# JINXER000/GIE-mapping

Measured on AMD Instinct MI355X. Metric: edt_map_update_throughput, higher is better.
Workload: dtype int32; 1 GPU; 512x512x512 @ 0.05 m, sensor-less hash world (BASELINE config 5): occupied iff hash(x,y,z) < 1 %, full observation, 25 ~; preset=c5, fast_mode=False, tiles=single volume, blocks=360448

## Files before the change

gie-mapping_amd/csrc/gie_hip.hip:

```cpp
#include <cstdio>
#include <unistd.h>
#include <cstring>
#include <cstdlib>
#include <string>
#include <algorithm>
#include <vector>
#include <hip/hip_runtime.h>
#include <hip/hip_ext.h>
#include <rocprim/rocprim.hpp>
#include "gie_kernels.hip.h"

#define GIE_NEV 8

struct be_state {
    int device;
    int num_cu;
    int cu_total;
    hipStream_t stream;
    hipEvent_t ev[GIE_NEV];
    int ev_set[GIE_NEV];
    void *scan_tmp; size_t scan_bytes;
    void *arena;
    hipEvent_t copy_ev[2];
    hipStream_t side;
// ... 267 lines not shown
}
static void be_exclusive_scan(be_state *b, const int32_t *flag, int32_t *rank, int n)
{
    size_t bytes = 0;
    (void)hipSetDevice(b->device);
    GIE_HIP_OK(rocprim::exclusive_scan(nullptr, bytes, flag, rank, 0, (size_t)n, rocprim::plus<int32_t>(), b->stream));
    if (bytes > b->scan_bytes) {
        if (b->scan_tmp) { (void)hipStreamSynchronize(b->stream); (void)hipFree(b->scan_tmp); }
        GIE_HIP_OK(hipMalloc(&b->scan_tmp, bytes)); b->scan_bytes = bytes;
    }
    GIE_HIP_OK(rocprim::exclusive_scan(b->scan_tmp, bytes, flag, rank, 0, (size_t)n, rocprim::plus<int32_t>(), b->stream));
}

template <int CP, int TX, int WAVES> static void gie_launch_edt_z(be_state *b, const gie_ctx &c, int full)
{
    constexpr int LP = 64 * CP;
    const size_t tile = ((size_t)c.Z * (TX + 1) + 3) & ~(size_t)3;
    const size_t lds = tile * 4 + (size_t)WAVES * LP * 8 + (size_t)LP * 2 + 16;
    static bool attr_done = false;
    if (!attr_done) {
        GIE_HIP_OK(hipFuncSetAttribute(reinterpret_cast<const void *>(&k_edt_z<CP, TX, WAVES>), hipFuncAttributeMaxDynamicSharedMemorySize, 160 * 1024));
        attr_done = true;
    }
    const int ntx = (c.X + TX - 1) / TX, ntiles = ntx * c.Y;
    int wgs = (int)((160 * 1024) / (lds + 256));
    if (wgs < 1) wgs = 1; if (wgs > 4) wgs = 4;
    int grid = wgs * b->cu_total; if (grid > (ntiles + 1) / 2) grid = (ntiles + 1) / 2;
    GIE_LAUNCH(b, (k_edt_z<CP, TX, WAVES>), dim3(grid), dim3(64 * WAVES), lds, c, ntx, ntiles, full);
}
template <int CP> static void gie_launch_edt_xz(be_state *b, const gie_ctx &c, bool zpass, int full, int zs_fused = 0, bool redo = false)
{
    if (redo) {
        GIE_LAUNCH(b, k_edt_x_redo<CP>, dim3(b->cu_total * 8), dim3(64 * GIE_EDTX_WAVES), 0, c);
    } else if (!zpass) {
        GIE_LAUNCH(b, k_edt_x<CP>, dim3((c.Y + GIE_EDTX_WAVES - 1) / GIE_EDTX_WAVES, c.Z), dim3(64 * GIE_EDTX_WAVES), 0, c, zs_fused, full);
    } else {
        gie_launch_edt_z<CP, 16, 8>(b, c, full);
    }
}
static void gie_launch_edt_dim(be_state *b, const gie_ctx &c, int L, bool zpass, int full, int zs_fused = 0, bool redo = false)
{
    if (L <= 64) gie_launch_edt_xz<1>(b, c, zpass, full, zs_fused, redo);
    else if (L <= 128) gie_launch_edt_xz<2>(b, c, zpass, full, zs_fused, redo);
    else if (L <= 256) gie_launch_edt_xz<4>(b, c, zpass, full, zs_fused, redo);
    else if (L <= 512) gie_launch_edt_xz<8>(b, c, zpass, full, zs_fused, redo);
    else gie_launch_edt_xz<16>(b, c, zpass, full, zs_fused, redo);
}
static int be_zs_mode(const gie_ctx &c)
{
    if (c.Z < 64 || c.Z > 1024) return 0;
    static const int on = GIE_SWITCH("GIE_ZSTREAM", 1);
    static const int fused = GIE_SWITCH("GIE_ZS_FUSED", 1);
    return on ? ((fused && (c.X & 1) == 0) ? 2 : 1) : 0;
}
static int be_edt_z_stream(be_state *b, const gie_ctx &c, int full);
static void be_edt_z_rest(be_state *b, const gie_ctx &c, int full, int zs)
{
    if (zs == 2) gie_launch_edt_dim(b, c, c.X, false, full, 0, true);
    gie_launch_edt_dim(b, c, c.Z, true, full);
}
static void be_edt_z(be_state *b, const gie_ctx &c, int full) { be_edt_z_rest(b, c, full, be_edt_z_stream(b, c, full) ? be_zs_mode(c) : 0); }
template <bool STAGED, class F> static void be_vox_list(be_state *b, const gie_ctx &c, const F &f, const int32_t *list, int count_idx, int always_list, int lx = 64)
{
    static const int mult = GIE_SWITCH("GIE_VOXA_MULT", 32);
    const dim3 g(b->cu_total * mult), t(256);
    if (lx == 32) GIE_LAUNCH(b, (k_voxa<F, STAGED, 32>), g, t, 0, c, f, list, count_idx, always_list);
    else if (lx == 16) GIE_LAUNCH(b, (k_voxa<F, STAGED, 16>), g, t, 0, c, f, list, count_idx, always_list);
    else if (lx == 8) GIE_LAUNCH(b, (k_voxa<F, STAGED, 8>), g, t, 0, c, f, list, count_idx, always_list);
    else GIE_LAUNCH(b, (k_voxa<F, STAGED, 64>), g, t, 0, c, f, list, count_idx, always_list);
}
static void be_markc(be_state *b, const gie_ctx &c, const int32_t *list)
{
    static const int generic = GIE_SWITCH("GIE_MARKC_GENERIC", 0);
    static const int lx = GIE_SWITCH("GIE_MARKC_LX", 32);
    static const int mult = GIE_SWITCH("GIE_VOXA_MULT", 64);
    if (generic) { be_vox_list<true>(b, c, op_markc(), list, GIE_CNT_TL_KNOWN, 0, lx == 16 || lx == 8 || lx == 32 ? lx : 64); return; }
    static const int lmult = GIE_SWITCH("GIE_MARKC_LGRID", 40);
    const dim3 g(b->cu_total * ((c.coc_defer && c.lazy_ok) ? lmult : mult)), t(256);
    if (lx == 16) GIE_LAUNCH(b, k_markc<16>, g, t, 0, c, list);
    else if (lx == 64) GIE_LAUNCH(b, k_markc<64>, g, t, 0, c, list);
    else GIE_LAUNCH(b, k_markc<32>, g, t, 0, c, list);
}
static float be_place_probe(be_state *b, const gie_ctx &c, int reps, int streams = 15)
{
    static const int mult = GIE_SWITCH("GIE_VOXA_MULT", 64);
    const long long ntile = (long long)c.tfd[0] * c.tfd[1] * c.tfd[2];
    const int nslot = (int)(ntile < c.max_blocks ? ntile : c.max_blocks);
    hipEvent_t e0, e1;
    if (hipEventCreate(&e0) != hipSuccess || hipEventCreate(&e1) != hipSuccess) return -1.f;
    std::vector<float> ms;
    hipLaunchKernelGGL(k_place_probe, dim3(b->cu_total * mult), dim3(256), 0, b->stream, c, nslot, streams);
    for (int r = 0; r < reps; r++) {
        (void)hipEventRecord(e0, b->stream);
        hipLaunchKernelGGL(k_place_probe, dim3(b->cu_total * mult), dim3(256), 0, b->stream, c, nslot, streams);
        (void)hipEventRecord(e1, b->stream);
        (void)hipEventSynchronize(e1);
        float t = 0.f; (void)hipEventElapsedTime(&t, e0, e1); ms.push_back(t);
    }
    (void)hipEventDestroy(e0); (void)hipEventDestroy(e1);
    std::sort(ms.begin(), ms.end());
    GIE_HIP_OK(hipMemsetAsync(c.pair, 0, (size_t)c.N * sizeof(uint64_t), b->stream));
    return ms.empty() ? -1.f : ms[ms.size() / 2];
}
static int be_rows_mode() { static const int v = GIE_SWITCH("GIE_ROWS", 1); return v ? 2 : 0; }
static void be_fuse(be_state *b, const gie_ctx &c, const int32_t *list)
{
    static const int mult = GIE_SWITCH("GIE_ROWS_MULT", 32);
    if (be_rows_mode()) {
        if (c.pntcld_mode) GIE_LAUNCH(b, k_fuse_rows<true>, dim3(b->cu_total * mult), dim3(256), 0, c, op_fuse(), list);
        else GIE_LAUNCH(b, k_fuse_rows<false>, dim3(b->cu_total * mult), dim3(256), 0, c, op_fuse(), list);
    }
    else be_vox_list<true>(b, c, op_fuse(), list, GIE_CNT_TL_FUSE, 0);
}
static void be_frontier_tiles(be_state *b, const gie_ctx &c, const int32_t *known, int known_idx, const int32_t *list, int count_idx)
{
    gie_face_patches fp;
    const int da[6] = { c.Y, c.Y, c.X, c.X, c.X, c.X }, db[6] = { c.Z, c.Z, c.Z, c.Z, c.Y, c.Y };
    fp.off[0] = 0;
    for (int f = 0; f < 6; f++) { fp.na[f] = (da[f] + 7) / 8; fp.off[f + 1] = fp.off[f] + fp.na[f] * ((db[f] + 7) / 8); }
    const long long ntile = (long long)c.tfd[0] * c.tfd[1] * c.tfd[2];
    int nsum = (int)((ntile + 64 * GIE_FF_WAVES - 1) / (64 * GIE_FF_WAVES));
    if (nsum > 2 * b->cu_total) nsum = 2 * b->cu_total;
    const int nface = (fp.off[6] + GIE_FF_WAVES - 1) / GIE_FF_WAVES;
    GIE_LAUNCH(b, k_frontier_faces, dim3(nsum + nface), dim3(64 * GIE_FF_WAVES), 0, c, fp, known, known_idx, nsum);
    static int mult = GIE_SWITCH("GIE_FRONT_MULT", 0);
    if (mult <= 0) {
        int per_cu = 0;
        if (hipOccupancyMaxActiveBlocksPerMultiprocessor(&per_cu, reinterpret_cast<const void *>(&k_frontier_tiles), 64 * GIE_FR_WAVES, 0) != hipSuccess || per_cu < 1) per_cu = 2;
        mult = per_cu;
    }
    GIE_LAUNCH(b, k_frontier_tiles, dim3(b->cu_total * mult), dim3(64 * GIE_FR_WAVES), 0, c, list, count_idx);
}
static void be_edt_z_direct(be_state *b, const gie_ctx &c)
{
    GIE_LAUNCH(b, k_edt_z_direct, dim3(b->cu_total * 16), dim3(256), 0, c);
}
static int be_edt_z_stream(be_state *b, const gie_ctx &c, int full)
{
    const int zs = be_zs_mode(c);
    if (!zs) return 0;
    const int nxr = (c.X + 63) / 64;
    static const int target = GIE_SWITCH("GIE_ZSTREAM_WAVES", 8);
    const long long want = (long long)b->cu_total * 4 * target;
    int nseg = (int)((want + (long long)nxr * c.Y - 1) / ((long long)nxr * c.Y));
    const int maxseg = c.Z / 64 > 0 ? c.Z / 64 : 1;
    if (nseg > maxseg) nseg = maxseg; if (nseg < 1) nseg = 1;
    int seg_len = ((c.Z + nseg - 1) / nseg + 31) & ~31;
    nseg = (c.Z + seg_len - 1) / seg_len;
    const long long waves = (long long)nxr * nseg * c.Y;
    long long grid = (waves + 3) / 4;
    const long long cap = (long long)b->cu_total * 8 * 4;
    if (grid > cap) grid = cap;
    if (!full && grid < (long long)b->cu_total * 16) grid = (long long)b->cu_total * 16;
    if (zs == 2) GIE_LAUNCH(b, k_edt_z_stream<true>, dim3((unsigned)grid), dim3(256), 0, c, full, nseg, seg_len, zs);
    else GIE_LAUNCH(b, k_edt_z_stream<false>, dim3((unsigned)grid), dim3(256), 0, c, full, nseg, seg_len, zs);
    return 1;
}
static void be_tile_oldskip(be_state *b, const gie_ctx &c, const int pupvt[3])
{
    const int ntile = c.tfd[0] * c.tfd[1] * c.tfd[2];
    int32_t *const count = &c.cnt[GIE_CNT_STATE1];
    GIE_LAUNCH(b, k_tile_oldskip, dim3((ntile + 255) / 256), dim3(256), 0, c, ntile, c.wc_list[0], count);
    if (c.catchup_fast) GIE_LAUNCH(b, k_coc_catchup_new, dim3(b->cu_total * 8), dim3(256), 0, c, pupvt[0], pupvt[1], pupvt[2], c.wc_list[0], count);
}
static void be_pair_materialise(be_state *b, const gie_ctx &c, int stay)
{
    const int ntile = c.tfd[0] * c.tfd[1] * c.tfd[2];
    int32_t *const count = &c.cnt[GIE_CNT_STATE2];
    GIE_LAUNCH(b, k_pair_lazy_list, dim3((ntile + 255) / 256), dim3(256), 0, c, ntile, stay, c.wc_list[1], count);
    GIE_LAUNCH(b, k_pair_lazy_run, dim3(b->cu_total * 8), dim3(256), 0, c, c.wc_list[1], count);
}
static void be_coc_catchup(be_state *b, const gie_ctx &c, const gie_catchup &p)
{
    const int ntile = c.tfd[0] * c.tfd[1] * c.tfd[2];
    int32_t *const count = &c.cnt[GIE_CNT_STATE1];
    GIE_HIP_OK(hipMemsetAsync(count, 0, sizeof(int32_t), b->stream));
    GIE_LAUNCH(b, k_coc_catchup_list, dim3((ntile + 255) / 256), dim3(256), 0, c, p, ntile, c.wc_list[0], count);
    GIE_LAUNCH(b, k_coc_catchup_run, dim3(b->cu_total * 4), dim3(256), 0, c, p, c.wc_list[0], count);
}
static void be_edt_prep(be_state *b, const gie_ctx &c)
{
    const int ncol = c.tfd[0] * c.tfd[1];
    GIE_LAUNCH(b, k_edt_prep, dim3((ncol + GIE_PREP_WAVES - 1) / GIE_PREP_WAVES), dim3(64 * GIE_PREP_WAVES), 0, c, ncol);
}
static void be_edt(be_state *b, const gie_ctx &c, int full)
{
    dim3 gy((c.X + GIE_EDTY_COLS - 1) / GIE_EDTY_COLS, c.Z);
    be_prof(b, 6, 0);
    static const int y4 = GIE_SWITCH("GIE_EDTY4", 1);
    if (y4 && (c.X & 3) == 0) {
        const int yb = c.Y > 512 ? 32 : 16, nq = (c.Y + yb - 1) / yb;
        const int lanes = (y4 == 3) ? 32 : 16;
        dim3 g4((c.X / 4 + lanes - 1) / lanes, c.Z), b4(lanes, nq);
        if (yb == 16 && lanes == 16) GIE_LAUNCH(b, (k_edt_y4<16, 16>), g4, b4, 0, c);
        else if (yb == 16) GIE_LAUNCH(b, (k_edt_y4<16, 32>), g4, b4, 0, c);
        else if (lanes == 16) GIE_LAUNCH(b, (k_edt_y4<32, 16>), g4, b4, 0, c);
        else GIE_LAUNCH(b, (k_edt_y4<32, 32>), g4, b4, 0, c);
    }
    else if (c.Y <= 256) GIE_LAUNCH(b, (k_edt_y<8, 8>), gy, dim3(GIE_EDTY_COLS, 8), 0, c);
    else if (c.Y <= 512) GIE_LAUNCH(b, (k_edt_y<16, 16>), gy, dim3(GIE_EDTY_COLS, 16), 0, c);
    else GIE_LAUNCH(b, (k_edt_y<32, 16>), gy, dim3(GIE_EDTY_COLS, 16), 0, c);
    be_prof(b, 6, 1);
    const int zs = be_zs_mode(c);
    be_prof(b, 7, 0); gie_launch_edt_dim(b, c, c.X, false, full, zs == 2 ? zs : 0); be_prof(b, 7, 1);
    be_prof(b, 8, 0);
    const int zl = be_edt_z_stream(b, c, full);
    if (!zl && !full) be_edt_z_direct(b, c);
    be_edt_z_rest(b, c, full, zl ? zs : 0);
    be_prof(b, 8, 1);

}
template <class F> static void be_chained(be_state *b, const F &enqueue)
{
    std::lock_guard<std::mutex> lock(g_waves_mutex);
    const int dv = b->device & 63;
    (void)hipSetDevice(b->device);
    const bool chain = g_live_mappers[dv] > 1;
    if (chain) {
        if (g_waves_event_set[dv]) GIE_HIP_OK(hipStreamWaitEvent(b->stream, g_waves_event[dv], 0));
        else { GIE_HIP_OK(hipEventCreateWithFlags(&g_waves_event[dv], hipEventDisableTiming)); g_waves_event_set[dv] = true; }
    }
    enqueue();
    if (chain) GIE_HIP_OK(hipEventRecord(g_waves_event[dv], b->stream));
}
static void be_waves(be_state *b, const gie_ctx &c, int with_ab, int record_seeds, int clear_first)
{
    be_chained(b, [&]() {
        if (clear_first) {
            GIE_HIP_OK(hipMemsetAsync(&c.cnt[GIE_CNT_BAR_B], 0, 2 * sizeof(int32_t), b->stream));
            GIE_HIP_OK(hipMemsetAsync(c.lvl_next, 0, 2 * GIE_MAX_LEVELS * sizeof(int32_t), b->stream));
        }
        if (with_ab) GIE_LAUNCH(b, k_waves_ab, dim3(b->num_cu), dim3(GIE_WAVE_THREADS), 0, c);
        GIE_LAUNCH(b, k_waves_c, dim3(b->num_cu), dim3(GIE_WAVE_THREADS), 0, c, with_ab, record_seeds);
    });
}

#include "gie_api.inc.h"
#include "gie_sdf.inc.h"
#include "gie_nf1.inc.h"
#include "gie_frontier.inc.h"
#include "gie_los.inc.h"
```

gie-mapping_amd/csrc/gie_kernels.hip.h:

```cpp
#ifndef GIE_KERNELS_HIP_H
#define GIE_KERNELS_HIP_H

#include <hip/hip_runtime.h>
#include "gie_functors.h"

#if defined(GIE_WAVE_TIMING) || defined(GIE_RAY_TIMING)
#include "../../tools/measure/gie_timing.h"
#endif
#if !defined(GIE_WAVE_TIMING)
#define GIE_TS2(tag, n) do { } while (0)
#define GIE_WPROF_DECL do { } while (0)
#define GIE_WPROF_MARK(base) do { } while (0)
#define GIE_WPROF_ADD(i, v) do { } while (0)
#define GIE_WPROF_END(base) do { } while (0)
#define GIE_WPROF_DRAIN() do { } while (0)
#define GIE_WPROF_SUB(i) do { } while (0)
#define GIE_WPROF_SUBSTART() do { } while (0)
#define GIE_WPROF_DUMP() do { } while (0)
#define GIE_WPROF_CLK() 0ull
#define GIE_WAVE_TIMING_RESET(cond) do { } while (0)
#endif
#if !defined(GIE_RAY_TIMING)
#define GIE_RTS(k) do { } while (0)
#endif
// ... 912 lines not shown
        for (int half = 0; half < 2; half++) {
            const int col = wave + 8 * half;
            const int x = x0 + col;
            if (x >= X) break;
            const uint64_t nc = half ? nd1 : nd0;
            if (nc == 0ull) continue;
            if (CP >= 4 && K > GIE_BAND_MAXK) {
                unsigned bn = 0;
#pragma unroll
                for (int m = 0; m < CP && m < 8; m++) if ((nc >> (8 * m)) & 0xffull) bn |= 1u << m;
                if (full) bn = ~0u;
                uint32_t *sk = reinterpret_cast<uint32_t *>(ce) + GIE_WIN_MAX;
#pragma unroll
                for (int m = 0; m < CP; m++) {
                    const int i = 64 * m + lane;
                    uint32_t key = GIE_WIN_NONE;
                    if ((zvalid >> m) & 1u) {
                        const uint32_t v = tile[i * TS + col];
                        if (v != 0xffffffffu) { const int dx = x - (int)(v & 0xffffu), dy = y - (int)(v >> 16); key = ((uint32_t)(dx * dx + dy * dy) << 10) | (uint32_t)i; }
                    }
                    sk[i] = key;
                }
                if (lane < GIE_WIN_MAX) { sk[-1 - lane] = GIE_WIN_NONE; sk[LP + lane] = GIE_WIN_NONE; }
                gie_wave_sync();
                uint32_t best[CP];
                const bool okw = gie_row_window<CP>(sk, Z, lane, best, bn);
                if (okw) {
                    uint32_t oc[CP];
#pragma unroll
                    for (int m = 0; m < CP; m++) {
                        if (64 * m + lane < Z && ((bn >> m) & 1u)) {
                            const int s = (int)(best[m] & 1023u);
                            const uint32_t v = tile[s * TS + col];
                            oc[m] = gie_pack_bcoc((int)(v & 0xffffu), (int)(v >> 16), s);
                        }
                    }
                    gie_wave_sync();
#pragma unroll
                    for (int m = 0; m < CP; m++)
                        if (64 * m + lane < Z && ((bn >> m) & 1u)) tile[(64 * m + lane) * TS + col] = oc[m];
                    gie_wave_sync();
                    continue;
                }
                gie_wave_sync();
            }
            for (int j = lane; j < K; j += 64) {
                const int i = s_zl[j];
                const uint32_t v = tile[i * TS + col];
                const int dx = x - (int)(v & 0xffffu), dy = y - (int)(v >> 16);
                ce[j] = make_uint2(((uint32_t)(dx * dx + dy * dy) << 10) | (uint32_t)j, (uint32_t)i << 5);
            }
            gie_wave_sync();
            if (K == 0) {
                for (int i = lane; i < Z; i += 64) tile[i * TS + col] = GIE_BCOC_NONE;
            } else {
                unsigned bandneed = 0;
#pragma unroll
                for (int m = 0; m < CP && m < 8; m++) if ((nc >> (8 * m)) & 0xffull) bandneed |= 1u << m;
                if (full) bandneed = ~0u;
                int sj[CP];
                const bool banded = K <= GIE_BAND_MAXK;
                if (banded) gie_row_argmin_banded<CP>(ce, K, Z, lane, sj, bandneed);
                else gie_row_argmin<CP>(ce, K, Z, lane, sj);
                const int ub = banded ? lane : lane * CP, us = banded ? 64 : 1;
                uint32_t oc[CP];
#pragma unroll
                for (int m = 0; m < CP; m++) {
                    if (ub + m * us < Z && (!banded || ((bandneed >> m) & 1u))) {
                        const int s = (int)((ce[sj[m]].y & 0xffffu) >> 5);
                        const uint32_t v = tile[s * TS + col];
                        oc[m] = gie_pack_bcoc((int)(v & 0xffffu), (int)(v >> 16), s);
                    }
                }
                gie_wave_sync();
#pragma unroll
                for (int m = 0; m < CP; m++)
                    if (ub + m * us < Z && (!banded || ((bandneed >> m) & 1u))) tile[(ub + m * us) * TS + col] = oc[m];
            }
            gie_wave_sync();
        }
        __syncthreads();
        {
            const int x = x0 + tx;
            {
                const unsigned voff = tzoff_b + (unsigned)(y * X + x) * 4u;
                static_assert(ZSTEP % 8 == 0, "a thread's rows are whole z tiles apart");
                const uint64_t nds = ((tx >> 3) ? nd1 : nd0) >> (tz >> 3);
                unsigned wm = 0;
#pragma unroll
                for (int j = 0; j < NLD; j++) if (full || (j * (ZSTEP / 8) < 64 && ((nds >> (j * (ZSTEP / 8))) & 1ull))) wm |= 1u << j;
                {
                    unsigned zl = zin;
                    asm volatile("" : "+v"(zl));
                    wm &= zl;
                    if (x >= X) wm = 0;
                }
                {
#pragma unroll
                    for (int j0 = 0; j0 < NLD; j0 += 4) {
                        uint32_t ov[4];
#pragma unroll
                        for (int u = 0; u < 4; u++) ov[u] = (j0 + u < NLD) ? tile[(tz + (j0 + u) * ZSTEP) * TS + tx] : 0u;
#pragma unroll
                        for (int u = 0; u < 4; u++) if (j0 + u < NLD) __builtin_amdgcn_raw_buffer_store_b32(ov[u], rs_out, ((wm >> (j0 + u)) & 1u) ? voff : GIE_BUF_OOB, (j0 + u) * zstride_b, 0);
                    }
                }
            }
        }
        __syncthreads();
    }
}

#ifndef GIE_ZS_R
#define GIE_ZS_R 8
#endif
#ifndef GIE_ZS_C
#define GIE_ZS_C 16
#endif
#define GIE_ZS_W (GIE_ZS_C + 2 * GIE_ZS_R)
#define GIE_ZS_LDAUX 2
#define GIE_ZS_STAUX 2
#define GIE_ZS_NONE 0xb0000000u
#define GIE_ZS_LIMIT ((uint32_t)((GIE_ZS_R + 1) * (GIE_ZS_R + 1)) << 24)
__device__ __forceinline__ uint32_t gie_zs_key(const uint32_t v, const bool plane_ok, const int x8, const int y8, const int j)
{
    const uint32_t ux = (uint32_t)(x8 - (int)(v & 0xffffu)), uy = (uint32_t)(y8 - (int)(v >> 16));
    const int dx = (int)ux - 8, dy = (int)uy - 8;
    const uint32_t a = (uint32_t)(__mul24(dx, dx) + __mul24(dy, dy));
    const bool ok = plane_ok && max(ux, uy) <= 16u && a < (uint32_t)((GIE_ZS_R + 1) * (GIE_ZS_R + 1));
    return ok ? ((a << 24) | ((uint32_t)j << 18) | (ux << 13) | (uy << 8)) : (GIE_ZS_NONE | ((uint32_t)j << 18));
}
#define GIE_ZS_XW (64 + 2 * GIE_ZS_R)
#define GIE_ZS_ROWS 8
#ifndef GIE_ZS_CHAINS
#define GIE_ZS_CHAINS 4
#endif
#ifndef GIE_ZS_FUSED_WGS
#define GIE_ZS_FUSED_WGS 7
#endif
__device__ __forceinline__ uint32_t gie_zs_col(const uint32_t cy, const bool ok, const int y8)
{
    const uint32_t uy = (uint32_t)(y8 - (int)cy);
    const int dy = (int)uy - 8;
    return (ok && uy <= 16u) ? (((uint32_t)__mul24(dy, dy) << 24) | (uy << 8)) : GIE_ZS_NONE;
}
typedef __attribute__((address_space(3))) uint32_t gie_lds_u32;
__device__ __forceinline__ uint32_t gie_zs_fused_key(const gie_lds_u32 *row, const int j)
{
    uint32_t m = 0xffffffffu;
#pragma unroll
    for (int k = 0; k <= 2 * GIE_ZS_R; k++) m = min(m, row[k] + (((uint32_t)((k - GIE_ZS_R) * (k - GIE_ZS_R)) << 24) | ((uint32_t)(15 + k) << 13)));
    return m < GIE_ZS_LIMIT ? ((m ^ (31u << 13)) | ((uint32_t)j << 18)) : (GIE_ZS_NONE | ((uint32_t)j << 18));
}
template <int NP, int JB, int AUX>
__device__ __forceinline__ void gie_zs_fused_keys(uint32_t (&wk)[GIE_ZS_W], uint32_t (*srow)[GIE_ZS_XW], const __amdgpu_buffer_rsrc_t rs, const unsigned vo,
                                                  const unsigned ps2, const int zfirst, const int Z, const unsigned long long pm, const bool ok0, const bool ok1, const int y8, const int lane)
{
    static_assert(NP % GIE_ZS_ROWS == 0, "whole batches of rows");
    uint32_t v[NP];
#pragma unroll
    for (int j = 0; j < NP; j++) {
        const unsigned so = (unsigned)min(max(__builtin_amdgcn_readfirstlane(zfirst) + j, 0), Z - 1) * ps2;
        v[j] = __builtin_amdgcn_raw_buffer_load_b32(rs, vo, so, AUX);
    }
#pragma unroll
    for (int j0 = 0; j0 < NP; j0 += GIE_ZS_ROWS) {
#pragma unroll
        for (int j = j0; j < j0 + GIE_ZS_ROWS; j++) {
            const bool po = (pm >> j) & 1ull;
            if (lane < GIE_ZS_XW / 2)
                *reinterpret_cast<uint2 *>(&srow[j - j0][2 * lane]) = make_uint2(gie_zs_col(v[j] & 0xffffu, po && ok0, y8), gie_zs_col(v[j] >> 16, po && ok1, y8));
        }
        gie_wave_sync();
        gie_lds_u32 *rp[GIE_ZS_CHAINS];
#pragma unroll
        for (int q = 0; q < GIE_ZS_CHAINS; q++) rp[q] = (gie_lds_u32 *)&srow[0][lane];
#pragma unroll
        for (int j = j0; j < j0 + GIE_ZS_ROWS; j++) {
            wk[JB + j] = gie_zs_fused_key(rp[j % GIE_ZS_CHAINS] + (j - j0) * GIE_ZS_XW, JB + j);
            asm volatile("" : "+v"(rp[j % GIE_ZS_CHAINS]) : "v"(wk[JB + j]));
        }
        gie_wave_sync();
    }
}
__device__ __forceinline__ void gie_edt_z_direct_body(const gie_ctx &c);
#define GIE_ZS_R2 24
__device__ __noinline__ bool gie_zs_wide_trip(const uint32_t *cxy2, uint32_t *bcoc, const unsigned nbytes, const unsigned voff, const unsigned pstride,
                                              const int zc, const int z1, const int Z, const int x, const int y, const bool inx, const uint8_t *occ)
{
    const __amdgpu_buffer_rsrc_t rs_in = __builtin_amdgcn_make_buffer_rsrc(const_cast<uint32_t *>(cxy2), 0, nbytes, 0x00020000);
    const __amdgpu_buffer_rsrc_t rs_out = __builtin_amdgcn_make_buffer_rsrc(bcoc, 0, nbytes, 0x00020000);
    uint32_t best[GIE_ZS_C];
#pragma unroll
    for (int t = 0; t < GIE_ZS_C; t++) best[t] = 0xffffffffu;
    const int lo = max(zc - GIE_ZS_R2, 0), hi = min(zc + GIE_ZS_C + GIE_ZS_R2, Z);
#pragma unroll 1
    for (int i0 = lo; i0 < hi; i0 += 8) {
        uint32_t v[8];
#pragma unroll
        for (int k = 0; k < 8; k++) v[k] = __builtin_amdgcn_raw_buffer_load_b32(rs_in, voff, (unsigned)min(i0 + k, Z - 1) * pstride, 0);
#pragma unroll
        for (int k = 0; k < 8; k++) {
            const int i = i0 + k;
            if (i >= hi || !occ[i]) continue;
            const int dx = x - (int)(v[k] & 0xffffu), dy = y - (int)(v[k] >> 16);
            const uint32_t a = (v[k] == 0xffffffffu) ? 0x3fffffu : (uint32_t)(dx * dx + dy * dy);
#pragma unroll
            for (int t = 0; t < GIE_ZS_C; t++) { const int d = zc + t - i; best[t] = min(best[t], (min(a + (uint32_t)(d * d), 0x3fffffu) << 10) | (uint32_t)i); }
        }
    }
    uint32_t worst = 0;
#pragma unroll
    for (int t = 0; t < GIE_ZS_C; t++) if (zc + t < z1) worst = max(worst, best[t]);
    if (__any(inx && worst >= ((uint32_t)((GIE_ZS_R2 + 1) * (GIE_ZS_R2 + 1)) << 10))) return false;
#pragma unroll
    for (int t = 0; t < GIE_ZS_C; t++) {
        const int sp = (int)(best[t] & 1023u);
        const uint32_t v = __builtin_amdgcn_raw_buffer_load_b32(rs_in, voff, (unsigned)sp * pstride, 0);
        __builtin_amdgcn_raw_buffer_store_b32(gie_pack_bcoc((int)(v & 0xffffu), (int)(v >> 16), sp), rs_out, (zc + t < z1) ? voff : GIE_BUF_OOB, (unsigned)min(zc + t, Z - 1) * pstride, 0);
    }
    return true;
}
#define GIE_ZS_XW2 (64 + 2 * GIE_ZS_R2)
static_assert(2 * GIE_ZS_XW2 <= GIE_ZS_ROWS * GIE_ZS_XW, "the wide trip's row and its cy fit the wave's LDS rows");
__device__ __forceinline__ bool gie_zs_wide_trip_fused(const __amdgpu_buffer_rsrc_t rs_cy, const __amdgpu_buffer_rsrc_t rs_out, gie_lds_u32 *srow, const unsigned voff,
                                                       const unsigned pstride, const unsigned ps2, const int zc, const int z1, const int Z, const int x0, const int x,
                                                       const int y, const int X, const uint8_t *occ, const int lane)
{
    const int xa = x0 - GIE_ZS_R2 + lane, xb = x0 + 64 - GIE_ZS_R2 + lane;
    const bool oka = xa >= 0 && xa < X, okb = lane < 2 * GIE_ZS_R2 && xb < X;
    const unsigned voa = oka ? (unsigned)(y * X + xa) * 2u : GIE_BUF_OOB, vob = okb ? (unsigned)(y * X + xb) * 2u : GIE_BUF_OOB;
    gie_lds_u32 *sq = srow, *scy = srow + GIE_ZS_XW2;
    uint32_t best[GIE_ZS_C], bc[GIE_ZS_C];
#pragma unroll
    for (int t = 0; t < GIE_ZS_C; t++) { best[t] = 0xffffffffu; bc[t] = GIE_BCOC_NONE; }
    const int lo = max(zc - GIE_ZS_R2, 0), hi = min(zc + GIE_ZS_C + GIE_ZS_R2, Z);
#pragma unroll 1
    for (int i0 = lo; i0 < hi; i0 += 8) {
        uint16_t va[8], vb[8];
#pragma unroll
        for (int k = 0; k < 8; k++) {
            const unsigned so = (unsigned)min(i0 + k, Z - 1) * ps2;
            va[k] = __builtin_amdgcn_raw_buffer_load_b16(rs_cy, voa, so, 0);
            vb[k] = __builtin_amdgcn_raw_buffer_load_b16(rs_cy, vob, so, 0);
        }
#pragma unroll
        for (int k = 0; k < 8; k++) {
            const int i = i0 + k;
            if (i >= hi || !occ[i]) continue;
            {
                const int da = y - (int)va[k], db = y - (int)vb[k];
                sq[lane] = (oka && va[k] != 0xffffu) ? ((uint32_t)(da * da) << 6) : 0x3fffffc0u; scy[lane] = va[k];
                if (lane < 2 * GIE_ZS_R2) { sq[64 + lane] = (okb && vb[k] != 0xffffu) ? ((uint32_t)(db * db) << 6) : 0x3fffffc0u; scy[64 + lane] = vb[k]; }
            }
            gie_wave_sync();
            uint32_t m = 0xffffffffu;
#pragma unroll
            for (int q = 0; q <= 2 * GIE_ZS_R2; q++) m = min(m, sq[lane + q] + (((uint32_t)((q - GIE_ZS_R2) * (q - GIE_ZS_R2)) << 6) | (uint32_t)q));
            const int q = (int)(m & 63u);
            const uint32_t cc = gie_pack_bcoc(x - GIE_ZS_R2 + q, (int)scy[lane + q], i);
            gie_wave_sync();
            const uint32_t a = min(m >> 6, 0x3fffffu);
#pragma unroll
            for (int t = 0; t < GIE_ZS_C; t++) {
                const int d = zc + t - i;
                const uint32_t nb = (min(a + (uint32_t)(d * d), 0x3fffffu) << 10) | (uint32_t)i;
                if (nb < best[t]) { best[t] = nb; bc[t] = cc; }
            }
        }
    }
    uint32_t worst = 0;
#pragma unroll
    for (int t = 0; t < GIE_ZS_C; t++) if (zc + t < z1) worst = max(worst, best[t]);
    if (__any(x < X && worst >= ((uint32_t)((GIE_ZS_R2 + 1) * (GIE_ZS_R2 + 1)) << 10))) return false;
#pragma unroll
    for (int t = 0; t < GIE_ZS_C; t++)
        __builtin_amdgcn_raw_buffer_store_b32(bc[t], rs_out, (zc + t < z1) ? voff : GIE_BUF_OOB, (unsigned)min(zc + t, Z - 1) * pstride, 0);
    return true;
}
template <bool FUSED>
__global__ __launch_bounds__(256, FUSED ? GIE_ZS_FUSED_WGS : 6) void k_edt_z_stream(const gie_ctx c, const int full, const int nseg, const int seg_len, const int zs)
{
    __shared__ uint8_t s_occ[1024 + 2 * (32 + 2 * GIE_ZS_R)];
    const int Z = c.Z, X = c.X, Y = c.Y;
    if (full == 0 && gie_z_use_lists(c, c.cnt[GIE_CNT_TL_KNOWN])) { gie_edt_z_direct_body(c); return; }
    if (!gie_zs_takes(c, zs, full)) return;
    __shared__ __attribute__((aligned(16))) uint32_t s_row[FUSED ? 4 : 1][FUSED ? GIE_ZS_ROWS : 1][GIE_ZS_XW];
    if (blockIdx.x == 0 && threadIdx.x == 0) c.cnt[GIE_CNT_ZSTREAM] = 1;
    for (int i = threadIdx.x; i < Z + 2 * GIE_ZS_W; i += 256) { const int z = i - GIE_ZS_W; s_occ[i] = (z >= 0 && z < Z) ? c.zocc[z] : (uint8_t)0; }
    __syncthreads();
    const int lane = threadIdx.x & 63;
    const int nxr = (X + 63) >> 6;
    const int total = nxr * nseg * Y;
    const size_t plane = (size_t)X * Y;
    const unsigned nbytes = (unsigned)((size_t)X * Y * Z * 4u);
    const __amdgpu_buffer_rsrc_t rs_in = __builtin_amdgcn_make_buffer_rsrc(const_cast<uint32_t *>(c.cxy2), 0, nbytes, 0x00020000);
    const __amdgpu_buffer_rsrc_t rs_cy = __builtin_amdgcn_make_buffer_rsrc(const_cast<uint16_t *>(c.cy1), 0, nbytes / 2u, 0x00020000);
    const __amdgpu_buffer_rsrc_t rs_out = __builtin_amdgcn_make_buffer_rsrc(c.bcoc, 0, nbytes, 0x00020000);
    const unsigned pstride = (unsigned)(plane * 4u), pstride2 = (unsigned)(plane * 2u);
    for (int w = (int)blockIdx.x * 4 + (int)(threadIdx.x >> 6); w < total; w += (int)gridDim.x * 4) {
        const int wu = __builtin_amdgcn_readfirstlane(w);
        const int xr = wu % nxr, seg = (wu / nxr) % nseg, y = wu / (nxr * nseg);
        const int x = xr * 64 + lane;
        const int z0 = seg * seg_len, z1 = min(Z, z0 + seg_len);
        if (z0 >= Z) continue;
        const unsigned voff = x < X ? (unsigned)(y * X + x) * 4u : GIE_BUF_OOB;
        const int x8 = x + 8, y8 = y + 8;
        uint32_t wk[GIE_ZS_W];
        const int xa = xr * 64 - GIE_ZS_R + 2 * lane;
        const bool oka = lane < GIE_ZS_XW / 2 && xa >= 0 && xa < X, okb = lane < GIE_ZS_XW / 2 && xa + 1 >= 0 && xa + 1 < X;
        const unsigned vpa = (oka || okb) ? (unsigned)(y * X + xa) * 2u : GIE_BUF_OOB;
        uint32_t (*srow)[GIE_ZS_XW] = s_row[FUSED ? (threadIdx.x >> 6) : 0];
        if (FUSED) {
            const int zz = z0 - GIE_ZS_R + lane;
            const unsigned long long pm = __ballot(lane < 2 * GIE_ZS_R && s_occ[zz + GIE_ZS_W] != 0);
            gie_zs_fused_keys<2 * GIE_ZS_R, 0, 0>(wk, srow, rs_cy, vpa, pstride2, z0 - GIE_ZS_R, Z, pm, oka, okb, y8, lane);
        } else {
            const int zz = z0 - GIE_ZS_R + lane;
            const unsigned long long pm = __ballot(lane < 2 * GIE_ZS_R && s_occ[zz + GIE_ZS_W] != 0);
            uint32_t v[2 * GIE_ZS_R];
#pragma unroll
            for (int j = 0; j < 2 * GIE_ZS_R; j++) { const int zp = min(max(z0 - GIE_ZS_R + j, 0), Z - 1); v[j] = __builtin_amdgcn_raw_buffer_load_b32(rs_in, voff, (unsigned)zp * pstride, 0); }
#pragma unroll
            for (int j = 0; j < 2 * GIE_ZS_R; j++) wk[j] = gie_zs_key(v[j], (pm >> j) & 1ull, x8, y8, j);
        }
        bool failed = false;
        int wide = 0, wz0 = 0, wz1 = 0;
#pragma unroll 1
        for (int zc = z0; zc < z1; zc += GIE_ZS_C) {
            if (FUSED) {
                const int zz = zc + GIE_ZS_R + lane;
                const unsigned long long pm = __ballot(lane < GIE_ZS_C && s_occ[zz + GIE_ZS_W] != 0);
                gie_zs_fused_keys<GIE_ZS_C, 2 * GIE_ZS_R, GIE_ZS_LDAUX>(wk, srow, rs_cy, vpa, pstride2, zc + GIE_ZS_R, Z, pm, oka, okb, y8, lane);
            } else {
                const int zz = zc + GIE_ZS_R + lane;
                const unsigned long long pm = __ballot(lane < GIE_ZS_C && s_occ[zz + GIE_ZS_W] != 0);
                uint32_t v[GIE_ZS_C];
#pragma unroll
                for (int j = 0; j < GIE_ZS_C; j++) { const int zp = min(zc + GIE_ZS_R + j, Z - 1); v[j] = __builtin_amdgcn_raw_buffer_load_b32(rs_in, voff, (unsigned)zp * pstride, GIE_ZS_LDAUX); }
#pragma unroll
                for (int j = 0; j < GIE_ZS_C; j++) wk[2 * GIE_ZS_R + j] = gie_zs_key(v[j], (pm >> j) & 1ull, x8, y8, 2 * GIE_ZS_R + j);
            }
            uint32_t wlo = 0, whi = 0;
#pragma unroll
            for (int t = 0; t < GIE_ZS_C; t++) {
                const int p = GIE_ZS_R + t;
                uint32_t b = wk[p];
#pragma unroll
                for (int d = 1; d <= GIE_ZS_R; d++) b = min(b, min(wk[p - d], wk[p + d]) + ((uint32_t)(d * d) << 24));
                const bool in = zc + t < z1;
                if (in) { if (t < 8) wlo = max(wlo, b); else whi = max(whi, b); }
                const int s = zc - GIE_ZS_R + (int)((b >> 18) & 63u);
                const int cx = x8 - (int)((b >> 13) & 31u), cy = y8 - (int)((b >> 8) & 31u);
                __builtin_amdgcn_raw_buffer_store_b32(gie_pack_bcoc(cx, cy, s), rs_out, in ? voff : GIE_BUF_OOB, (unsigned)min(zc + t, Z - 1) * pstride, GIE_ZS_STAUX);
            }
            const uint32_t worst = max(wlo, whi);
            {
                static_assert(GIE_ZS_C == 16, "a trip is two tiles high");
                uint32_t m0 = x < X ? (wlo >> 24) : 0u, m1 = x < X ? (whi >> 24) : 0u;
                m0 = max(m0, (uint32_t)__shfl_xor((int)m0, 1)); m1 = max(m1, (uint32_t)__shfl_xor((int)m1, 1));
                m0 = max(m0, (uint32_t)__shfl_xor((int)m0, 2)); m1 = max(m1, (uint32_t)__shfl_xor((int)m1, 2));
                m0 = max(m0, (uint32_t)__shfl_xor((int)m0, 4)); m1 = max(m1, (uint32_t)__shfl_xor((int)m1, 4));
                if ((lane & 7) == 0 && x < X) {
                    const int t0 = gie_tile_index(c, x, y, zc);
                    __hip_atomic_fetch_max(&c.tbmax[t0], (int32_t)m0, __ATOMIC_RELAXED, __HIP_MEMORY_SCOPE_AGENT);
                    if (zc + 8 < z1) __hip_atomic_fetch_max(&c.tbmax[t0 + c.tfd[0] * c.tfd[1]], (int32_t)m1, __ATOMIC_RELAXED, __HIP_MEMORY_SCOPE_AGENT);
                }
            }
            if (__any(x < X && worst >= GIE_ZS_LIMIT)) {
                if (wide == 2) { failed = true; break; }
                if (wide == 0) wz0 = zc; else wz1 = zc;
                wide++;
            }
#pragma unroll
            for (int j = 0; j < 2 * GIE_ZS_R; j++) wk[j] = wk[GIE_ZS_C + j] - ((uint32_t)GIE_ZS_C << 18);
        }
        if (wide > 0 && lane == 0) atomicAdd(&c.cnt[GIE_CNT_ZWIDE], wide);
        if (FUSED) {
#pragma unroll 1
            for (int k = 0; k < wide && !failed; k++)
                failed = !gie_zs_wide_trip_fused(rs_cy, rs_out, (gie_lds_u32 *)&srow[0][0], voff, pstride, pstride2, __builtin_amdgcn_readfirstlane(k ? wz1 : wz0), z1, Z, xr * 64, x, y, X,
                                                 s_occ + GIE_ZS_W, lane);
        } else {
            if (!failed && wide > 0) failed = !gie_zs_wide_trip(c.cxy2, c.bcoc, nbytes, voff, pstride, wz0, z1, Z, x, y, x < X, s_occ + GIE_ZS_W);
            if (!failed && wide > 1) failed = !gie_zs_wide_trip(c.cxy2, c.bcoc, nbytes, voff, pstride, wz1, z1, Z, x, y, x < X, s_occ + GIE_ZS_W);
        }
        if (failed) {
            if (lane < 4) {
                const int tx16 = xr * 4 + lane;
                if (tx16 * 16 < X) c.zredo[(size_t)y * ((X + 15) >> 4) + tx16] = 1u;
                if (lane == 0) atomicAdd(&c.cnt[GIE_CNT_ZFAIL], 1);
            }
            if ((lane & 7) == 0 && x < X)
                for (int zt = z0; zt < z1; zt += 8) __hip_atomic_fetch_max(&c.tbmax[gie_tile_index(c, x, y, zt)], (int32_t)((GIE_ZS_R + 1) * (GIE_ZS_R + 1)), __ATOMIC_RELAXED, __HIP_MEMORY_SCOPE_AGENT);
        }
    }
}

#define GIE_PREP_WAVES 16
__global__ __launch_bounds__(64 * GIE_PREP_WAVES) void k_edt_prep(const gie_ctx c, const int ncol)
{
    if (blockIdx.x == 0 && threadIdx.x < 64) {
        uint8_t f[16];
#pragma unroll
        for (int i = 0; i < 16; i++) { const int z = 64 * i + (int)threadIdx.x; f[i] = c.zocc[min(z, c.Z - 1)]; }
        int k = 0;
#pragma unroll
        for (int i = 0; i < 16; i++) {
            const int z = 64 * i + (int)threadIdx.x;
            const bool v = z < c.Z && f[i];
            const unsigned long long m = __ballot(v);
            if (v) c.zlist[k + __popcll(m & ((1ull << threadIdx.x) - 1ull))] = (uint16_t)z;
            k += __popcll(m);
        }
        if (threadIdx.x == 0) *c.zcount = k;
    }
    const int col = blockIdx.x * GIE_PREP_WAVES + (threadIdx.x >> 6);
    const bool colok = col < ncol;
    const int tx = colok ? col % c.tfd[0] : 0, ty = colok ? col / c.tfd[0] : 0;
    for (int tz0 = 0; tz0 < c.tfd[2]; tz0 += 64) {
        const int tz = tz0 + (int)(threadIdx.x & 63);
        const int t = (tz * c.tfd[1] + ty) * c.tfd[0] + tx;
        const bool k = colok && tz < c.tfd[2] && c.tknown[t];
        const unsigned long long m = __ballot(k);
        if (colok && tz == 0) c.zneed[col] = m;
        const int slot = gie_wg_reserve(&c.cnt[GIE_CNT_TL_KNOWN], k);
        if (slot >= 0) c.tl_known[slot] = t;
        const int slot2 = gie_wg_reserve(&c.cnt[GIE_CNT_TL_SWEPT], k && c.tskip[t] != 2);
        if (slot2 >= 0) c.tl_swept[slot2] = t;
    }
}

__global__ __launch_bounds__(256) void k_tile_oldskip(const gie_ctx c, const int ntile, int32_t *list, int32_t *count)
{
    int any = 0;
    for (int z = threadIdx.x; z < c.Z; z += 256) any |= c.zocc[z];
    any = __syncthreads_or(any);
    const int t = blockIdx.x * 256 + threadIdx.x;
    bool need = false;
    if (t < ntile) need = gie_tile_oldskip(c, t, any) != 0;
    const int slot = gie_wg_reserve(count, need);
    if (slot >= 0) list[slot] = t;
}
__global__ __launch_bounds__(256) void k_coc_catchup_new(const gie_ctx c, const int pu0, const int pu1, const int pu2, const int32_t *list, const int32_t *count)
{
    const int n = *count;
    const int lane = threadIdx.x & 63;
    const int pupvt[3] = { pu0, pu1, pu2 };
    for (int e = (int)blockIdx.x * 4 + (int)(threadIdx.x >> 6); e < n; e += (int)gridDim.x * 4) gie_coc_catchup_newcolumn(c, pupvt, list[e], lane);
}

__global__ __launch_bounds__(256) void k_pair_lazy_list(const gie_ctx c, const int ntile, const int stay, int32_t *list, int32_t *count)
{
    const int t = blockIdx.x * 256 + threadIdx.x;
    const bool need = t < ntile && c.tlazy[t] != 0 && !(stay && c.tskip[t] == 2);
    const int slot = gie_wg_reserve(count, need);
    if (slot >= 0) list[slot] = t;
}
__global__ __launch_bounds__(256) void k_pair_lazy_run(const gie_ctx c, const int32_t *list, const int32_t *count)
{
    const int n = *count;
    const int lane = threadIdx.x & 63;
    for (int e = (int)blockIdx.x * 4 + (int)(threadIdx.x >> 6); e < n; e += (int)gridDim.x * 4) {
        const int t = list[e];
        gie_pair_materialise_column(c, t, lane);
        if (lane == 0) c.tlazy[t] = 0;
    }
}

__global__ __launch_bounds__(256) void k_coc_catchup_list(const gie_ctx c, const gie_catchup p, const int ntile, int32_t *list, int32_t *count)
{
    const int t = blockIdx.x * 256 + threadIdx.x;
    const bool need = t < ntile && gie_coc_catchup_tile(c, p, t);
    const int slot = gie_wg_reserve(count, need);
    if (slot >= 0) list[slot] = t;
}
__global__ __launch_bounds__(256) void k_coc_catchup_run(const gie_ctx c, const gie_catchup p, const int32_t *list, const int32_t *count)
{
    const int n = *count;
    const int lane = threadIdx.x & 63;
    for (int e = (int)blockIdx.x * 4 + (int)(threadIdx.x >> 6); e < n; e += (int)gridDim.x * 4) gie_coc_catchup_column(c, p, list[e], lane);
}

template <class F, bool STAGED>
__device__ __forceinline__ void gie_vox_column(const gie_ctx &c, const F &f, const int x, const int y, const int z0)
{
// ... 1836 lines not shown
```

Before: 100,600 Mvoxels/s.

## Pack two z-planes per LDS word and run the fused x-scan on packed 16-bit lanes

Adds a packed form of the fused z-stream key builder, enabled by default through GIE_ZS_PACKED. Pairs of planes are interleaved as 16-bit halves in LDS, and the x-window min is computed with packed u16x2 min/add. The full key is then rebuilt from a separate byte table of y offsets. This aims to halve LDS traffic and ALU work in the inner min loop and to shrink the per-wave LDS row footprint, which could raise occupancy. The cost is extra permute and decode work, plus tighter encoding limits on 16-bit lanes that have to stay exact.

```diff
diff --git a/gie-mapping_amd/csrc/gie_hip.hip b/gie-mapping_amd/csrc/gie_hip.hip
--- a/gie-mapping_amd/csrc/gie_hip.hip
+++ b/gie-mapping_amd/csrc/gie_hip.hip
@@ -443,8 +443,10 @@
     const long long cap = (long long)b->cu_total * 8 * 4;
     if (grid > cap) grid = cap;
     if (!full && grid < (long long)b->cu_total * 16) grid = (long long)b->cu_total * 16;
-    if (zs == 2) GIE_LAUNCH(b, k_edt_z_stream<true>, dim3((unsigned)grid), dim3(256), 0, c, full, nseg, seg_len, zs);
-    else GIE_LAUNCH(b, k_edt_z_stream<false>, dim3((unsigned)grid), dim3(256), 0, c, full, nseg, seg_len, zs);
+    static const int packed = GIE_SWITCH("GIE_ZS_PACKED", 1);
+    if (zs == 2 && packed) GIE_LAUNCH(b, k_edt_z_stream<2>, dim3((unsigned)grid), dim3(256), 0, c, full, nseg, seg_len, zs);
+    else if (zs == 2) GIE_LAUNCH(b, k_edt_z_stream<1>, dim3((unsigned)grid), dim3(256), 0, c, full, nseg, seg_len, zs);
+    else GIE_LAUNCH(b, k_edt_z_stream<0>, dim3((unsigned)grid), dim3(256), 0, c, full, nseg, seg_len, zs);
     return 1;
 }
 static void be_tile_oldskip(be_state *b, const gie_ctx &c, const int pupvt[3])
diff --git a/gie-mapping_amd/csrc/gie_kernels.hip.h b/gie-mapping_amd/csrc/gie_kernels.hip.h
--- a/gie-mapping_amd/csrc/gie_kernels.hip.h
+++ b/gie-mapping_amd/csrc/gie_kernels.hip.h
@@ -1088,11 +1088,37 @@
     for (int k = 0; k <= 2 * GIE_ZS_R; k++) m = min(m, row[k] + (((uint32_t)((k - GIE_ZS_R) * (k - GIE_ZS_R)) << 24) | ((uint32_t)(15 + k) << 13)));
     return m < GIE_ZS_LIMIT ? ((m ^ (31u << 13)) | ((uint32_t)j << 18)) : (GIE_ZS_NONE | ((uint32_t)j << 18));
 }
-template <int NP, int JB, int AUX>
+#define GIE_ZS_PROWS (GIE_ZS_ROWS / 2 + GIE_ZS_ROWS / 4)
+#ifndef GIE_ZS_PCHAINS
+#define GIE_ZS_PCHAINS 2
+#endif
+typedef uint16_t gie_u16x2 __attribute__((ext_vector_type(2)));
+typedef __attribute__((address_space(3))) uint8_t gie_lds_u8;
+#define GIE_PK16(x) ((gie_u16x2)(uint16_t)(x))
+__device__ __forceinline__ uint32_t gie_zs_fused_pair(const gie_lds_u32 *row)
+{
+    gie_u16x2 m = GIE_PK16(0xffffu);
+#pragma unroll
+    for (int k = 0; k <= 2 * GIE_ZS_R; k++)
+        m = __builtin_elementwise_min(m, __builtin_bit_cast(gie_u16x2, (uint32_t)row[k]) + GIE_PK16((((k - GIE_ZS_R) * (k - GIE_ZS_R)) << 8) | k));
+    return __builtin_bit_cast(uint32_t, m);
+}
+template <bool HI>
+__device__ __forceinline__ uint32_t gie_zs_pair_key(const uint32_t m, const gie_lds_u8 *ut, const int j)
+{
+    const uint32_t k = HI ? ((m >> 16) & 31u) : (m & 31u);
+    uint32_t t = ut[k * 2u];
+    asm volatile("" : "+v"(t));
+    const uint32_t a = HI ? (m & 0xff000000u) : ((m & 0xff00u) << 16);
+    const uint32_t key = (uint32_t)((int)(a + (((uint32_t)j << 18) | (16u << 13) | (16u << 8))) + __mul24((int)k, -(1 << 13)) + __mul24((int)t, -(1 << 8)));
+    return a < GIE_ZS_LIMIT ? key : (GIE_ZS_NONE | ((uint32_t)j << 18));
+}
+template <int NP, int JB, int AUX, bool PACKED>
 __device__ __forceinline__ void gie_zs_fused_keys(uint32_t (&wk)[GIE_ZS_W], uint32_t (*srow)[GIE_ZS_XW], const __amdgpu_buffer_rsrc_t rs, const unsigned vo,
                                                   const unsigned ps2, const int zfirst, const int Z, const unsigned long long pm, const bool ok0, const bool ok1, const int y8, const int lane)
 {
     static_assert(NP % GIE_ZS_ROWS == 0, "whole batches of rows");
+    static_assert(GIE_ZS_ROWS == 8, "the packed rows: four plane pairs, two rows of y offsets");
     uint32_t v[NP];
 #pragma unroll
     for (int j = 0; j < NP; j++) {
@@ -1101,6 +1127,42 @@
     }
 #pragma unroll
     for (int j0 = 0; j0 < NP; j0 += GIE_ZS_ROWS) {
+        if (PACKED) {
+            const uint32_t lmask = (ok0 ? 0u : 0xffffu) | (ok1 ? 0u : 0xffff0000u);
+            gie_u16x2 d[GIE_ZS_ROWS], t[GIE_ZS_ROWS];
+#pragma unroll
+            for (int r = 0; r < GIE_ZS_ROWS; r++) {
+                const uint32_t smask = ((pm >> (j0 + r)) & 1ull) ? 0u : 0xffffffffu;
+                const gie_u16x2 cy = __builtin_elementwise_min(__builtin_bit_cast(gie_u16x2, v[j0 + r] | smask | lmask), GIE_PK16(0x7fffu));
+                t[r] = __builtin_elementwise_min(cy - GIE_PK16(y8 - 16), GIE_PK16(17));
+                const gie_u16x2 dy = GIE_PK16(8) - t[r];
+                d[r] = (dy * dy) << GIE_PK16(8);
+            }
+            if (lane < GIE_ZS_XW / 2) {
+#pragma unroll
+                for (int r = 0; r < GIE_ZS_ROWS; r += 2) {
+                    const uint32_t d0 = __builtin_bit_cast(uint32_t, d[r]), d1 = __builtin_bit_cast(uint32_t, d[r + 1]);
+                    const uint32_t t0 = __builtin_bit_cast(uint32_t, t[r]), t1 = __builtin_bit_cast(uint32_t, t[r + 1]);
+                    *reinterpret_cast<uint2 *>(&srow[r / 2][2 * lane]) = make_uint2(__builtin_amdgcn_perm(d1, d0, 0x05040100u), __builtin_amdgcn_perm(d1, d0, 0x07060302u));
+                    (&srow[GIE_ZS_ROWS / 2][0])[(r / 2) * (GIE_ZS_XW / 2) + lane] = __builtin_amdgcn_perm(t1, t0, 0x06020400u);
+                }
+            }
+            gie_wave_sync();
+            gie_lds_u32 *rp[GIE_ZS_PCHAINS];
+#pragma unroll
+            for (int q = 0; q < GIE_ZS_PCHAINS; q++) rp[q] = (gie_lds_u32 *)&srow[0][lane];
+            const gie_lds_u8 *const ut = (const gie_lds_u8 *)(gie_lds_u32 *)&srow[GIE_ZS_ROWS / 2][0] + 2 * lane;
+#pragma unroll
+            for (int r = 0; r < GIE_ZS_ROWS; r += 2) {
+                gie_lds_u32 *&base = rp[(r / 2) % GIE_ZS_PCHAINS];
+                const uint32_t m = gie_zs_fused_pair(base + (r / 2) * GIE_ZS_XW);
+                wk[JB + j0 + r] = gie_zs_pair_key<false>(m, ut + (r / 2) * (2 * GIE_ZS_XW), JB + j0 + r);
+                wk[JB + j0 + r + 1] = gie_zs_pair_key<true>(m, ut + (r / 2) * (2 * GIE_ZS_XW) + 1, JB + j0 + r + 1);
+                asm volatile("" : "+v"(base) : "v"(wk[JB + j0 + r]), "v"(wk[JB + j0 + r + 1]));
+            }
+            gie_wave_sync();
+            continue;
+        }
 #pragma unroll
         for (int j = j0; j < j0 + GIE_ZS_ROWS; j++) {
             const bool po = (pm >> j) & 1ull;
@@ -1158,7 +1220,7 @@
     return true;
 }
 #define GIE_ZS_XW2 (64 + 2 * GIE_ZS_R2)
-static_assert(2 * GIE_ZS_XW2 <= GIE_ZS_ROWS * GIE_ZS_XW, "the wide trip's row and its cy fit the wave's LDS rows");
+static_assert(2 * GIE_ZS_XW2 <= GIE_ZS_PROWS * GIE_ZS_XW, "the wide trip's row and its cy fit the wave's LDS rows (the packed form's: the fewer)");
 __device__ __forceinline__ bool gie_zs_wide_trip_fused(const __amdgpu_buffer_rsrc_t rs_cy, const __amdgpu_buffer_rsrc_t rs_out, gie_lds_u32 *srow, const unsigned voff,
                                                        const unsigned pstride, const unsigned ps2, const int zc, const int z1, const int Z, const int x0, const int x,
                                                        const int y, const int X, const uint8_t *occ, const int lane)
@@ -1214,14 +1276,15 @@
         __builtin_amdgcn_raw_buffer_store_b32(bc[t], rs_out, (zc + t < z1) ? voff : GIE_BUF_OOB, (unsigned)min(zc + t, Z - 1) * pstride, 0);
     return true;
 }
-template <bool FUSED>
-__global__ __launch_bounds__(256, FUSED ? GIE_ZS_FUSED_WGS : 6) void k_edt_z_stream(const gie_ctx c, const int full, const int nseg, const int seg_len, const int zs)
-{
+template <int FORM>
+__global__ __launch_bounds__(256, FORM ? GIE_ZS_FUSED_WGS : 6) void k_edt_z_stream(const gie_ctx c, const int full, const int nseg, const int seg_len, const int zs)
+{
+    constexpr bool FUSED = FORM != 0, PACKED = FORM == 2;
     __shared__ uint8_t s_occ[1024 + 2 * (32 + 2 * GIE_ZS_R)];
     const int Z = c.Z, X = c.X, Y = c.Y;
     if (full == 0 && gie_z_use_lists(c, c.cnt[GIE_CNT_TL_KNOWN])) { gie_edt_z_direct_body(c); return; }
     if (!gie_zs_takes(c, zs, full)) return;
-    __shared__ __attribute__((aligned(16))) uint32_t s_row[FUSED ? 4 : 1][FUSED ? GIE_ZS_ROWS : 1][GIE_ZS_XW];
+    __shared__ __attribute__((aligned(16))) uint32_t s_row[FUSED ? 4 : 1][FUSED ? (PACKED ? GIE_ZS_PROWS : GIE_ZS_ROWS) : 1][GIE_ZS_XW];
     if (blockIdx.x == 0 && threadIdx.x == 0) c.cnt[GIE_CNT_ZSTREAM] = 1;
     for (int i = threadIdx.x; i < Z + 2 * GIE_ZS_W; i += 256) { const int z = i - GIE_ZS_W; s_occ[i] = (z >= 0 && z < Z) ? c.zocc[z] : (uint8_t)0; }
     __syncthreads();
@@ -1250,7 +1313,7 @@
         if (FUSED) {
             const int zz = z0 - GIE_ZS_R + lane;
             const unsigned long long pm = __ballot(lane < 2 * GIE_ZS_R && s_occ[zz + GIE_ZS_W] != 0);
-            gie_zs_fused_keys<2 * GIE_ZS_R, 0, 0>(wk, srow, rs_cy, vpa, pstride2, z0 - GIE_ZS_R, Z, pm, oka, okb, y8, lane);
+            gie_zs_fused_keys<2 * GIE_ZS_R, 0, 0, PACKED>(wk, srow, rs_cy, vpa, pstride2, z0 - GIE_ZS_R, Z, pm, oka, okb, y8, lane);
         } else {
             const int zz = z0 - GIE_ZS_R + lane;
             const unsigned long long pm = __ballot(lane < 2 * GIE_ZS_R && s_occ[zz + GIE_ZS_W] != 0);
@@ -1267,7 +1330,7 @@
             if (FUSED) {
                 const int zz = zc + GIE_ZS_R + lane;
                 const unsigned long long pm = __ballot(lane < GIE_ZS_C && s_occ[zz + GIE_ZS_W] != 0);
-                gie_zs_fused_keys<GIE_ZS_C, 2 * GIE_ZS_R, GIE_ZS_LDAUX>(wk, srow, rs_cy, vpa, pstride2, zc + GIE_ZS_R, Z, pm, oka, okb, y8, lane);
+                gie_zs_fused_keys<GIE_ZS_C, 2 * GIE_ZS_R, GIE_ZS_LDAUX, PACKED>(wk, srow, rs_cy, vpa, pstride2, zc + GIE_ZS_R, Z, pm, oka, okb, y8, lane);
             } else {
                 const int zz = zc + GIE_ZS_R + lane;
                 const unsigned long long pm = __ballot(lane < GIE_ZS_C && s_occ[zz + GIE_ZS_W] != 0);
```

Result: slower. 95150 Mvoxels/s (-5.4%).
